# AnimatedRNG/alphazero-rs

Measured on AMD Instinct MI355X. Metric: selfplay_games_per_sec, higher is better.
Workload: dtype bf16

## Files before the change

alphazero-rs_amd/csrc/az_engine.hip:

```cpp
#include "../../include/az_engine.h"
#include "../../include/az_reanalyse.h"
#include "../../include/az_search_stop.h"

#include <dlfcn.h>
#include <unistd.h>
#include <rccl/rccl.h>

#include <algorithm>
#include <array>
#include <atomic>
#include <chrono>
#include <cstdio>
#include <cstring>
#include <map>
#include <memory>
#include <mutex>
#include <string>
#include <vector>

#include "az_combine.h"
#include "az_draw.h"
#include "az_local_comm.h"
#include "az_merge.h"
#include "az_net.h"
// ... 1120 lines not shown
    if (is("train_epochs") && value >= 1 && value <= 100000) { e->train_epochs = (int)value; return AZ_OK; }
    if (is("train_batch") && value >= 2 && value <= TRAIN_MAX_BATCH) { e->train_batch = (int)value; return AZ_OK; }
    if (is("train_seed")) { e->train_seed = (uint64_t)value; return AZ_OK; }
    if (is("train_graph") && (value == 0 || value == 1)) { e->train_graph = (int)value; if (e->trainer) trainer_set_graph(e->trainer, value != 0); return AZ_OK; }
    struct SwitchKey { const char* key; int TrainSwitches::* field; };
    static const SwitchKey switch_keys[] = {
        {"train_gemm", &TrainSwitches::gemm},
        {"train_fwd_dma", &TrainSwitches::fwd_dma},
        {"train_fwd_x3", &TrainSwitches::fwd_x3},
        {"train_wgrad_tr", &TrainSwitches::wgrad_tr},
        {"train_implicit", &TrainSwitches::implicit},
        {"train_gemm3_ring", &TrainSwitches::gemm3_ring},
        {"train_fork", &TrainSwitches::fork},
    };
    for (const SwitchKey& r : switch_keys) {
        if (!is(r.key) || (value != 0 && value != 1)) continue;
        e->train_sw.*r.field = (int)value;
        if (e->trainer) { (void)hipSetDevice(e->device); trainer_set_switches(e->trainer, e->train_sw); }
        return AZ_OK;
    }
    if (is("train_lr_e9") && value > 0) { e->hyper.lr = (float)((double)value * 1e-9); return AZ_OK; }
    if (is("train_dropout_e6") && value >= 0 && value < 1000000) { e->hyper.dropout = (float)((double)value * 1e-6); return AZ_OK; }
    if (is("train_keep_best") && (value == 0 || value == 1)) { e->train_keep_best = value; return AZ_OK; }
    if (is("train_patience")) {
        if (value < 0 || value > SCORE_MAX_PATIENCE) return fail(e, AZ_ERR_BAD_ARGUMENT, "train_patience must be in 0 .. 1000");
        e->train_patience = value;
        return AZ_OK;
    }
    struct OptimKey { const char* key; int64_t lo, hi; bool or_zero; int64_t az_engine::* field; const char* range; };
    static const OptimKey optim_keys[] = {
        {"train_weight_decay_e9", 0, OPTIM_WD_E9_MAX, false, &az_engine::train_weight_decay_e9, "train_weight_decay_e9 must be in 0 .. 1000000000"},
        {"train_clip_norm_e6", 1, OPTIM_CLIP_E6_MAX, true, &az_engine::train_clip_norm_e6, "train_clip_norm_e6 must be 0 or in 1 .. 1000000000000"},
        {"train_lr_warmup_steps", 0, OPTIM_STEPS_MAX, false, &az_engine::train_lr_warmup_steps, "train_lr_warmup_steps must be in 0 .. 2147483647"},
        {"train_lr_decay", 0, 2, false, &az_engine::train_lr_decay, "train_lr_decay must be 0, 1 or 2"},
        {"train_lr_floor_e6", 0, OPTIM_FLOOR_E6_MAX, false, &az_engine::train_lr_floor_e6, "train_lr_floor_e6 must be in 0 .. 1000000"},
        {"train_lr_total_steps", 0, OPTIM_STEPS_MAX, false, &az_engine::train_lr_total_steps, "train_lr_total_steps must be in 0 .. 2147483647"},
        {"train_ema_decay_e9", 1, OPTIM_EMA_E9_MAX, true, &az_engine::train_ema_decay_e9, "train_ema_decay_e9 must be 0 or in 1 .. 999999999"},
    };
    for (const OptimKey& r : optim_keys) {
        if (!is(r.key)) continue;
        if ((value < r.lo || value > r.hi) && !(r.or_zero && value == 0)) return fail(e, AZ_ERR_BAD_ARGUMENT, r.range);
        e->*r.field = value;
        return AZ_OK;
    }
#ifdef AZ_DIAG
    NetOptions& o = e->netopt;
    if (is("conv2_table") && value == 2) { o.conv2_table = 2; return AZ_OK; }
    if (is("gemm_variant") && (value == 0 || value == 1 || value == 2 || value == 3 || value == 5 || value == 13)) { o.gemm_variant = (int)value; return AZ_OK; }
    if (is("fc_ring") && value >= 0 && value <= 3) { o.fc_ring = (int)value; return AZ_OK; }
    if (is("ring_tile") && value >= 0 && value < 60000) { const int l = (int)(value / 10000); if (l >= 3 && l <= 5) o.ring_tile[l] = (int)(value % 10000); return AZ_OK; }
    if (is("conv3_ring") && value >= 0 && value <= 3) { o.conv3_ring = (int)value; return AZ_OK; }
    if (is("conv2_pipe") && (value == 0 || value == 1)) { o.conv2_pipe = (int)value; return AZ_OK; }
    if (is("conv3_pipe") && value >= 0 && value <= 3) { o.conv3_pipe = (int)value; return AZ_OK; }
    if (is("conv1_table") && (value == 0 || value == 1)) { o.conv1_table = (int)value; return AZ_OK; }
    if (is("conv4_big") && value >= 0 && value <= 2) { o.conv4_big = (int)value; return AZ_OK; }
    if (is("tree_stamps") && (value == 0 || value == 1)) { return tree_set_stamps((int)value) ? AZ_OK : fail(e, AZ_ERR_HIP, "tree_set_stamps"); }
    if (is("print_clock_stamps")) {
        auto it = e->nets.find((int)value);
        std::vector<unsigned long long> st(2048);
        if (it == e->nets.end() || !it->second.conv || !netws_read_clock_stamps(e->ws[0], st.data()))
            return fail(e, AZ_ERR_BAD_ARGUMENT, "no conv net under that model id");
        std::vector<double> mhz;
        for (int i = 0; i < 1024; ++i) if (st[2 * i + 1]) mhz.push_back(100.0 * (double)st[2 * i] / (double)st[2 * i + 1]);
        std::sort(mhz.begin(), mhz.end());
        if (mhz.empty()) return fail(e, AZ_ERR_BAD_ARGUMENT, "no stamps (run a forward with gemm_variant 13 first)");
        char buf[160];
        std::snprintf(buf, sizeof buf, "clock MHz min %.0f median %.0f max %.0f over %zu blocks", mhz.front(), mhz[mhz.size() / 2], mhz.back(), mhz.size());
        e->err = buf;
        return AZ_OK;
    }
    if (is("print_seg_stamps")) {
        std::vector<unsigned long long> st(2048);
        if (!e->ws[0] || !netws_read_clock_stamps(e->ws[0], st.data())) return fail(e, AZ_ERR_BAD_ARGUMENT, "no workspace");
        std::string out;
        for (int i = 0; i < 10; ++i) {
            std::vector<unsigned long long> v;
            for (int b = 0; b < 128; ++b) if (st[16 * b + 8]) v.push_back(st[16 * b + i]);
            if (v.empty()) return fail(e, AZ_ERR_BAD_ARGUMENT, "no stamps (run a forward with conv3_pipe 3 first)");
            std::sort(v.begin(), v.end());
            char buf[64];
            std::snprintf(buf, sizeof buf, "%s%llu", i ? " " : "", v[v.size() / 2]);
            out += buf;
        }
        e->err = out;
        return AZ_OK;
    }
    if (is("print_tree_stamps")) {
        std::vector<unsigned long long> st(4096 * 8);
        if (!tree_read_stamps(st.data())) return fail(e, AZ_ERR_BAD_ARGUMENT, "no stamps (set tree_stamps 1 and run a search first)");
        std::string out;
        for (int i = 0; i < 7; ++i) {
            std::vector<unsigned long long> v;
            for (int w = 0; w < 4096; ++w) if (st[(size_t)w * 8 + 6]) v.push_back(st[(size_t)w * 8 + i]);
            if (v.empty()) return fail(e, AZ_ERR_BAD_ARGUMENT, "no stamps yet");
            std::sort(v.begin(), v.end());
            char buf[96];
            std::snprintf(buf, sizeof buf, "%s%llu/%llu/%llu", i ? " " : "", v[v.size() / 10], v[v.size() / 2], v[v.size() * 9 / 10]);
            out += buf;
        }
        e->err = out;
        return AZ_OK;
    }
#else
    static const struct { const char* k; int64_t dflt; } diag_keys[] = {{"gemm_variant", 5}, {"fc_ring", 1}, {"conv3_ring", 0}, {"conv2_pipe", 1},
                                                                         {"conv3_pipe", 1}, {"conv1_table", 1}, {"conv4_big", 0}, {"tree_stamps", 0}};
    bool diag_key = is("print_clock_stamps") || is("print_seg_stamps") || is("print_tree_stamps") || (is("conv2_table") && value == 2);
// ... 2648 lines not shown
```

alphazero-rs_amd/csrc/az_net.h:

```cpp
#pragma once
#include "az_tree.h"

namespace az {

struct ConvNet;
struct NetWorkspace;

struct Layout {
    int C;
    int64_t conv_w[4], conv_b[4], conv_bn[4], fc_w[2], fc_b[2], fc_bn[2], pi_w, pi_b, v_w, v_b, total;
    explicit Layout(int c) : C(c) {
        int64_t o = 0;
        for (int l = 0; l < 4; ++l) {
            int cin = l == 0 ? 2 : C;
            conv_w[l] = o; o += 9ll * cin * C;
            conv_b[l] = o; o += C;
            conv_bn[l] = o; o += 4ll * C;
        }
        const int fin[2] = {6 * C, 1024}, fout[2] = {1024, 512};
        for (int l = 0; l < 2; ++l) {
            fc_w[l] = o; o += (int64_t)fin[l] * fout[l];
            fc_b[l] = o; o += fout[l];
            fc_bn[l] = o; o += 4ll * fout[l];
        }
        pi_w = o; o += 512 * 7; pi_b = o; o += 7;
        v_w = o; o += 512; v_b = o; o += 1;
        total = o;
    }
};


struct NetProfile {
    double conv2_ms = 0, conv2_flops = 0, total_ms = 0, total_flops = 0;
    double conv3_ms = 0, conv3_flops = 0;
    double conv4_ms = 0, conv4_flops = 0;
    double fc_ms = 0, fc_flops = 0;
    double rows = 0;
    double conv2_bytes = 0;
    uint64_t launches = 0;
};

void launch_net_fixture(const EvalBatch& eb, int kind, uint64_t salt, hipStream_t s);

ConvNet* convnet_create(int channels, const char** err);
void convnet_destroy(ConvNet* n);
NetWorkspace* netws_create(int channels, int max_batch, const char** err);
void netws_destroy(NetWorkspace* ws);
int64_t convnet_param_count(int channels);
bool convnet_set_params(ConvNet* n, const float* host_params, int64_t count);
bool convnet_get_params(const ConvNet* n, float* host_params, int64_t count);
void convnet_init_random(ConvNet* n, uint64_t seed);
void netws_resolve_profile(NetWorkspace* ws, NetProfile* prof);
bool netws_conv3_accounting(NetWorkspace* ws, unsigned long long out[2], bool reset);
struct NetOptions {
    int conv2_table = 1;
    int conv3_small = 1;
    int conv3_planes = 1;
    int ring_packed = 1;
    int conv3_tail = 1;
    int conv3_wreg = 1;
    int net_fp8 = 0;
    int narrow_rows = 32;
    int gemm_variant = 5;
    int conv1_table = 1;
    int conv2_pipe = 1;
    int conv3_pipe = 1;
    int conv3_ring = 0;
    int conv4_big = 0;
    int fc_ring = 1;
    int ring_tile[6] = {0, 0, 0, 0, 0, 0};
};
bool netws_read_clock_stamps(NetWorkspace* ws, unsigned long long* out2048);
long long netws_read_conv3_out(NetWorkspace* ws, int rows, void* out);
#ifdef AZ_DIAG
long long netws_read_act(NetWorkspace* ws, int layer, int rows, void* out);
long long convnet_read_conv_table(const ConvNet* n, int which, int first_row, int n_rows, void* out);
#endif
long long netws_read_conv3_out_fp8(NetWorkspace* ws, int rows, void* out);
long long netws_read_conv2_out_fp8(NetWorkspace* ws, int rows, void* out);
unsigned long long netws_fp8_skinny_launches(const NetWorkspace* ws);
bool convnet_build_fp8(ConvNet* n, NetWorkspace* ws, hipStream_t s);
bool convnet_fp8_scales(const ConvNet* n, float out[2]);
bool convnet_prepare(NetWorkspace* ws, const NetOptions& opt);
void convnet_forward(ConvNet* n, NetWorkspace* ws, const EvalBatch& eb, int n_rows_hint, int n_rows_typ, hipStream_t s, NetProfile* prof,
                     const NetOptions& opt);

}
```

alphazero-rs_amd/csrc/az_net.hip:

```cpp
#include "az_net.h"
#include "az_fp8.h"

#include <algorithm>
#include <cmath>
#include <cstring>
#include <vector>

namespace az {

constexpr int ACTIONS = ConnectFour::ACTIONS;

typedef __bf16 bf16x8 __attribute__((ext_vector_type(8)));
typedef float f32x4 __attribute__((ext_vector_type(4)));
typedef int i32x4 __attribute__((ext_vector_type(4)));
typedef int i32x8 __attribute__((ext_vector_type(8)));

__global__ void k_net_fixture(EvalBatch eb, int kind, uint64_t salt) {
    uint32_t i = blockIdx.x * blockDim.x + threadIdx.x;
    if (i >= *eb.n) return;
    float pi[ACTIONS], v;
    if (kind == 0) {
#pragma unroll
        for (int a = 0; a < ACTIONS; ++a) pi[a] = __fdiv_rn(1.0f, 7.0f);
        v = 1.0f;
// ... 715 lines not shown
                    const int rl = mt * 16 + frow;
                    float r0 = acc[mt][nt][0] + bv.x, r1 = acc[mt][nt][1] + bv.y, r2 = acc[mt][nt][2] + bv.z,
                          r3 = acc[mt][nt][3] + bv.w;
                    if (d.relu) { r0 = fmaxf(r0, 0.f); r1 = fmaxf(r1, 0.f); r2 = fmaxf(r2, 0.f); r3 = fmaxf(r3, 0.f); }
                    uint2 o;
                    o.x = pack_bf16x2(r0, r1);
                    o.y = pack_bf16x2(r2, r3);
                    *(uint2*)(smem + rl * EP_STRIDE + nl * 2) = o;
                }
            }
        }
        __syncthreads();
#pragma unroll
        for (int it = 0; it < 128 * 16 / 256; ++it) {
            const int idx = it * 256 + tid;
            const int rl = idx >> 4, c = idx & 15;
            const int ml = half * 128 + rl;
            const int m = b0 * 42 + ml;
            if (ml >= IMG_ROWS || m >= M) continue;
            *(uint4*)(d.out + (size_t)m * d.N + n0 + c * 8) = *(const uint4*)(smem + rl * EP_STRIDE + c * 16);
        }
        __syncthreads();
    }
}

constexpr int C3_PLANE_BYTES = 32768;
constexpr int C3_TAB_INV = 512;
constexpr int C3_TAB_RD = 9 * 2 * 16 * 8;
constexpr int WF3_STEP = 4096;
constexpr int WF3_PAD = 1;
constexpr int C3_NB = 12;

template <int NB, int IH, int IW, int MT, int NTW, bool PLANES = false, int WREG = 0>
struct ConvTile {
    static constexpr int OH = IH - 2, OW = IW - 2, OUT_PER = OH * OW, IN_PER = IH * IW;
    static constexpr int OUT_ROWS = NB * OUT_PER, IMG_R = NB * IN_PER;
    static constexpr int NCOL = 32 * NTW, WROWS = 16 * MT;
    static constexpr int IMG_BYTES = PLANES ? 2 * C3_PLANE_BYTES : (IMG_R * 128 + 1023) / 1024 * 1024;
    static constexpr int LDS_BYTES = IMG_BYTES + (WREG ? 0 : NCOL * 128);
    static constexpr int EP_STRIDE = NCOL * 2 + 16;
    static_assert(OUT_ROWS <= 2 * WROWS && IMG_R % 8 == 0 && MT % 2 == 0, "tile");
    static_assert(LDS_BYTES <= 81920, "two workgroups must fit a CU's 160 KiB");
    static_assert(OUT_ROWS * EP_STRIDE <= LDS_BYTES, "the output tile must fit the dead buffers");
};

template <int NB, int IH, int IW, int MT, int NTW, bool PLANES = false, int WREG = 0>
__device__ __forceinline__ void conv_valid_tile(const GemmDesc& d, unsigned char* smem, const int b0 , const int n0 ,
                                                const int n_boards) {
    using T = ConvTile<NB, IH, IW, MT, NTW, PLANES, WREG>;
    static_assert(!PLANES || (NB == C3_NB && IH == 6 && IW == 7 && MT == 8), "the cell maps are conv3's");
    constexpr int OUT_PER = T::OUT_PER, IN_PER = T::IN_PER, OUT_ROWS = T::OUT_ROWS, IMG_R = T::IMG_R, NCOL = T::NCOL, OW = T::OW;
    constexpr int IMG_BYTES = T::IMG_BYTES;
    constexpr int IPIECES = (IMG_R + 31) / 32, WPIECES = NCOL / 32;
    constexpr int MH = MT / 2;
    constexpr int NM = MH * NTW;
    const int M = n_boards * OUT_PER;
    const int C = d.cin;
    const int tid = threadIdx.x, lane = tid & 63;
    const int wave = __builtin_amdgcn_readfirstlane(tid >> 6);
    const int wr = wave >> 1, wc = wave & 1;
    const int lrow = lane >> 3;
    const int chunk = (lane & 7) ^ lrow;
    typedef __attribute__((address_space(3))) void* lds_ptr;
    const uint32_t i_ob = (uint32_t)((b0 * IN_PER + wave * 8 + lrow) * C + chunk * 8) * 2u;
    uint32_t i_obp[8];
    if constexpr (PLANES) {
#pragma unroll
        for (int j = 0; j < 8; ++j) {
            const uint32_t e = d.c3tab[j * 64 + wave * 16 + (lane >> 2)];
            i_obp[j] = (uint32_t)((b0 * IN_PER + (int)(e & 1023u)) * C + (int)((((uint32_t)lane & 3u) ^ ((e >> 10) & 3u)) << 4)) * 2u;
        }
    }
    const uint32_t w_ob = (uint32_t)((n0 + wave * 8 + lrow) * d.K + chunk * 8) * 2u;
    const uint32_t lds_img = (uint32_t)(uintptr_t)(lds_ptr)(smem + wave * 1024);
    const uint32_t lds_w = (uint32_t)(uintptr_t)(lds_ptr)(smem + IMG_BYTES + wave * 1024);
    const size_t i_stride = (size_t)64 * C, w_stride = (size_t)64 * d.K;
#define AZ_TDMA_W(kk_)                                                                                       \
    {                                                                                                        \
        const char* wbase = (const char*)(d.W + (kk_));                                                      \
        _Pragma("unroll") for (int q_ = 0; q_ < WPIECES; ++q_) lds_dma16(wbase + q_ * w_stride, w_ob, lds_w + q_ * 4096); \
    }
#define AZ_TDMA_IMG(cb_)                                                                                     \
    {                                                                                                        \
        const char* ibase = (const char*)(d.A + (cb_) * 64);                                                 \
        if constexpr (PLANES) {                                                                              \
            _Pragma("unroll") for (int q_ = 0; q_ < 16; ++q_) lds_dma16(ibase + (q_ >> 3) * 16, i_obp[q_ & 7], lds_img + q_ * 4096); \
        } else {                                                                                             \
            _Pragma("unroll") for (int q_ = 0; q_ < IPIECES; ++q_)                                           \
                if ((q_ * 4 + 3) * 8 + 7 < IMG_R || (q_ * 4 + wave) * 8 + 7 < IMG_R)                         \
                    lds_dma16(ibase + q_ * i_stride, i_ob, lds_img + q_ * 4096);                             \
        }                                                                                                    \
    }
    f32x4 acc[MT][NTW];
#pragma unroll
    for (int i = 0; i < MT; ++i)
#pragma unroll
        for (int jn = 0; jn < NTW; ++jn) acc[i][jn] = f32x4{0.f, 0.f, 0.f, 0.f};
    const int frow = lane & 15, fq = lane >> 4, fsw = lane & 7;
    int rbase[MT];
#pragma unroll
    for (int mt = 0; mt < MT; ++mt) {
        int ml = wr * T::WROWS + mt * 16 + frow;
        ml = ml < OUT_ROWS ? ml : 0;
        const int bl = ml / OUT_PER, p = ml - bl * OUT_PER, y = p / OW, x = p - y * OW;
        rbase[mt] = bl * IN_PER + y * IW + x;
    }
    const int b_row0 = IMG_BYTES + (wc * (16 * NTW) + frow) * 128;
    const int coffB0 = ((0 + fq) ^ fsw) << 4, coffB1 = ((4 + fq) ^ fsw) << 4;
    const uint4* rdtab = (const uint4*)(d.c3tab + C3_TAB_INV) + (wr * 16 + frow);
    const uint32_t lane_x = (((uint32_t)fq & 1u) << 15) | (((uint32_t)fq >> 1) << 4);
    uint32_t tq[4] = {0, 0, 0, 0}, ntq[4] = {0, 0, 0, 0};
    if constexpr (PLANES) { const uint4 v = rdtab[0]; tq[0] = v.x; tq[1] = v.y; tq[2] = v.z; tq[3] = v.w; }
#define AZ_TCELL(q_, mt_) ((((mt_) & 1) ? q_[(mt_) >> 1] >> 16 : q_[(mt_) >> 1] & 0xFFFFu) ^ lane_x)
#define AZ_TLDA(dst_, mt0_, ks_, dt_, q_)                                                                    \
    _Pragma("unroll") for (int i_ = 0; i_ < MH; ++i_) {                                                      \
        if constexpr (PLANES) {                                                                              \
            dst_[i_] = *(const bf16x8*)(smem + (AZ_TCELL(q_, (mt0_) + i_) ^ ((ks_) << 5)));                  \
        } else {                                                                                             \
            const int r_ = rbase[(mt0_) + i_] + (dt_);                                                       \
            dst_[i_] = *(const bf16x8*)(smem + r_ * 128 + ((((ks_) * 4 + fq) ^ (r_ & 7)) << 4));             \
        }                                                                                                    \
    }
#define AZ_TLDB(dst_, coff_)                                                                                 \
    _Pragma("unroll") for (int i_ = 0; i_ < NTW; ++i_)                                                       \
        dst_[i_] = *(const bf16x8*)(smem + b_row0 + i_ * 2048 + (coff_));
#define AZ_TMMA(mt0_, fb_, fa_)                                                                              \
    _Pragma("unroll") for (int i_ = 0; i_ < MH; ++i_)                                                        \
        _Pragma("unroll") for (int j_ = 0; j_ < NTW; ++j_)                                                   \
            acc[(mt0_) + i_][j_] = __builtin_amdgcn_mfma_f32_16x16x32_bf16(fb_[j_], fa_[i_], acc[(mt0_) + i_][j_], 0, 0, 0);
#define AZ_TSB __builtin_amdgcn_sched_barrier(0)
#define AZ_TMIX(nr_)                                                                                         \
    {                                                                                                        \
        constexpr int nmf_ = NM / (2 * (nr_)) > 1 ? NM / (2 * (nr_)) : 1;                                    \
        _Pragma("unroll") for (int g_ = 0; g_ < (nr_); ++g_) {                                               \
            __builtin_amdgcn_sched_group_barrier(0x008, nmf_, 0);                                            \
            __builtin_amdgcn_sched_group_barrier(0x100, 1, 0);                                               \
        }                                                                                                    \
        if (NM - nmf_ * (nr_) > 0) __builtin_amdgcn_sched_group_barrier(0x008, NM - nmf_ * (nr_), 0);        \
    }
    static_assert(NM >= NTW + MH, "a cluster must hold at least one MFMA per read of its region");
    bf16x8 faX[MH], faY[MH];
    const int ncb = C / 64;
    const int nk = ncb * 9;
    int cb = 0, tap = 0, dt = 0;
    if constexpr (WREG == 0) {
    AZ_TDMA_W(0);
    AZ_TDMA_IMG(0);
    asm volatile("s_waitcnt vmcnt(0)" ::: "memory");
    __syncthreads();
    bf16x8 fbX[NTW], fbY[NTW];
    AZ_TLDB(fbX, coffB0);
    AZ_TLDA(faX, 0, 0, 0, tq);
    for (int kt = 0; kt < nk; ++kt) {
        const bool sw = tap == 8;
        const int ntap = sw ? 0 : tap + 1, ncbi = sw ? cb + 1 : cb;
        const int nky = ntap / 3, ndt = nky * IW + (ntap - nky * 3);
        const int kk = kt + 1 < nk ? ntap * C + ncbi * 64 : 8 * C + cb * 64;
        if constexpr (PLANES) { const uint4 v = rdtab[ntap * 32]; ntq[0] = v.x; ntq[1] = v.y; ntq[2] = v.z; ntq[3] = v.w; }
        AZ_TLDB(fbY, coffB1);
        AZ_TLDA(faY, MH, 0, dt, tq);
        AZ_TMMA(0, fbX, faX);
        AZ_TMIX(NTW + MH);
        AZ_TSB;
        __builtin_amdgcn_s_waitcnt(0xC07F);
        __builtin_amdgcn_s_barrier();
        AZ_TSB;
        AZ_TDMA_W(kk);
        AZ_TLDA(faX, 0, 1, dt, tq);
        AZ_TMMA(MH, fbX, faY);
        AZ_TMIX(MH);
        AZ_TSB;
        AZ_TLDA(faY, MH, 1, dt, tq);
        AZ_TMMA(0, fbY, faX);
        AZ_TMIX(MH);
        AZ_TSB;
        __builtin_amdgcn_s_waitcnt(0xC07F);
        asm volatile("s_waitcnt vmcnt(0)" ::: "memory");
        __builtin_amdgcn_s_barrier();
        AZ_TSB;
        if (sw && ncbi < ncb) {
            AZ_TDMA_IMG(ncbi);
            asm volatile("s_waitcnt vmcnt(0)" ::: "memory");
            __builtin_amdgcn_s_barrier();
        }
        AZ_TSB;
        AZ_TLDB(fbX, coffB0);
        AZ_TLDA(faX, 0, 0, ndt, ntq);
        AZ_TMMA(MH, fbY, faY);
        AZ_TMIX(NTW + MH);
        AZ_TSB;
        tap = ntap; cb = ncbi; dt = ndt;
        if constexpr (PLANES) { tq[0] = ntq[0]; tq[1] = ntq[1]; tq[2] = ntq[2]; tq[3] = ntq[3]; }
    }
    } else {
        static_assert(PLANES && WREG == 1, "the ring needs the 64 KiB PLANES image (the epilogue's tile must fit it)");
        static_assert(NTW == 4 || NTW == 2, "a wave's columns are one 64-channel group of the packed copy, or half of one");
        const __amdgpu_buffer_rsrc_t wrs = __builtin_amdgcn_make_buffer_rsrc((void*)d.Wf, 0, (d.K * d.N + WF3_PAD * WF3_STEP) * 2, 0x00020000);
        uint32_t wfo = (uint32_t)(((n0 >> 6) + (NTW == 4 ? wc : 0)) * nk) * 8192u + (uint32_t)(NTW == 4 ? 0 : wc * 2) * 2048u;
        const uint32_t wlane = (uint32_t)lane * 16u;
        bf16x8 fwX[NTW], fwY[NTW];
#define AZ_TLDW(dst_, off_)                                                                                  \
    _Pragma("unroll") for (int j_ = 0; j_ < NTW; ++j_)                                                       \
        dst_[j_] = __builtin_bit_cast(bf16x8, __builtin_amdgcn_raw_buffer_load_b128(wrs, wlane, wfo + (uint32_t)((off_) + j_ * 2048), 0));
        AZ_TDMA_IMG(0);
        AZ_TLDW(fwX, 0);
        AZ_TLDW(fwY, 1024);
        asm volatile("s_waitcnt vmcnt(0)" ::: "memory");
        __syncthreads();
        AZ_TLDA(faX, 0, 0, 0, tq);
        for (int kt = 0; kt < nk; ++kt) {
            const bool sw = tap == 8;
            const int ntap = sw ? 0 : tap + 1, ncbi = sw ? cb + 1 : cb;
            const int nky = ntap / 3, ndt = nky * IW + (ntap - nky * 3);
            { const uint4 v = rdtab[ntap * 32]; ntq[0] = v.x; ntq[1] = v.y; ntq[2] = v.z; ntq[3] = v.w; }
            AZ_TLDA(faY, MH, 0, dt, tq);
            AZ_TMMA(0, fwX, faX);
            AZ_TMIX(MH);
            AZ_TSB;
            AZ_TLDA(faX, 0, 1, dt, tq);
            AZ_TMMA(MH, fwX, faY);
            AZ_TMIX(MH);
            AZ_TSB;
            AZ_TLDW(fwX, 8192);
            AZ_TLDA(faY, MH, 1, dt, tq);
            AZ_TMMA(0, fwY, faX);
            __builtin_amdgcn_sched_group_barrier(0x020, NTW, 0);
            AZ_TMIX(MH);
            AZ_TSB;
            if (sw && ncbi < ncb) {
                __builtin_amdgcn_s_waitcnt(0xC07F);
                __builtin_amdgcn_s_barrier();
                AZ_TDMA_IMG(ncbi);
                asm volatile("s_waitcnt vmcnt(0)" ::: "memory");
                __builtin_amdgcn_s_barrier();
            }
            AZ_TSB;
            AZ_TLDA(faX, 0, 0, ndt, ntq);
            AZ_TMMA(MH, fwY, faY);
            AZ_TMIX(MH);
            AZ_TSB;
            AZ_TLDW(fwY, 8192 + 1024);
            wfo += 8192u;
            AZ_TSB;
            tap = ntap; cb = ncbi; dt = ndt;
            tq[0] = ntq[0]; tq[1] = ntq[1]; tq[2] = ntq[2]; tq[3] = ntq[3];
        }
#undef AZ_TLDW
    }
#undef AZ_TDMA_W
#undef AZ_TDMA_IMG
#undef AZ_TLDA
#undef AZ_TCELL
#undef AZ_TLDB
#undef AZ_TMMA
#undef AZ_TSB
#undef AZ_TMIX
    constexpr int EP_STRIDE = T::EP_STRIDE;
    __builtin_amdgcn_s_waitcnt(0xC07F);
    __builtin_amdgcn_s_barrier();
#pragma unroll
    for (int nt = 0; nt < NTW; ++nt) {
        const int nl = wc * (16 * NTW) + nt * 16 + fq * 4;
        const float4 bv = *(const float4*)(d.bias + n0 + nl);
#pragma unroll
        for (int mt = 0; mt < MT; ++mt) {
            const int ml = wr * T::WROWS + mt * 16 + frow;
            if (ml >= OUT_ROWS) continue;
            float r0 = acc[mt][nt][0] + bv.x, r1 = acc[mt][nt][1] + bv.y, r2 = acc[mt][nt][2] + bv.z,
                  r3 = acc[mt][nt][3] + bv.w;
            if (d.relu) { r0 = fmaxf(r0, 0.f); r1 = fmaxf(r1, 0.f); r2 = fmaxf(r2, 0.f); r3 = fmaxf(r3, 0.f); }
            uint2 o;
            o.x = pack_bf16x2(r0, r1);
            o.y = pack_bf16x2(r2, r3);
            *(uint2*)(smem + ml * EP_STRIDE + nl * 2) = o;
        }
    }
    __syncthreads();
    constexpr int EP_CHUNKS = OUT_ROWS * (NCOL / 8);
#pragma unroll
    for (int it = 0; it < (EP_CHUNKS + 255) / 256; ++it) {
        const int idx = it * 256 + tid;
        const int ml = idx / (NCOL / 8), c = idx - ml * (NCOL / 8);
        const int m = b0 * OUT_PER + ml;
        if (idx >= EP_CHUNKS || m >= M) continue;
        *(uint4*)(d.out + (size_t)m * d.N + n0 + c * 8) = *(const uint4*)(smem + ml * EP_STRIDE + c * 16);
    }
}

constexpr int C3_TAIL = 128;
template <bool PLANES, int WREG>
__device__ __forceinline__ void conv3_auto_body(const GemmDesc& d, unsigned char* smem, const int full_grid, const int tail_wgs) {
    const int n_boards = (int)(*d.n_dev);
    if (n_boards * d.rows_per_sample <= d.m_min) return;
    if (blockIdx.x == 0 && threadIdx.x == 0 && d.acct && n_boards > 0) { atomicAdd(&d.acct[0], (unsigned long long)n_boards); atomicAdd(&d.acct[1], 1ull); }
    const int NT = d.N / 128;
    const int tiles8 = ((n_boards + C3_NB - 1) / C3_NB + 7) / 8 * 8;
    const int wid = tiles8 * NT;
    const int full_rounds = wid / 512 * 512, rem = wid - full_rounds;
    const bool cut = rem > 0 && rem <= tail_wgs;
    int id = blockIdx.x, half = -1;
    if (id >= full_grid) {
        if (!cut || id - full_grid >= rem) return;
        id = full_rounds + (id - full_grid);
        half = 1;
    } else if (cut && id >= full_rounds) {
        half = 0;
    }
    const int xcd = id & 7, j = id >> 3;
    const int ntile = j % NT, mtile = (j / NT) * 8 + xcd;
    const int b0 = mtile * C3_NB, n0 = ntile * 128;
    if (b0 >= n_boards) return;
    if (half < 0) conv_valid_tile<C3_NB, 6, 7, 8, 4, PLANES, WREG>(d, smem, b0, n0, n_boards);
    else conv_valid_tile<C3_NB, 6, 7, 8, 2, PLANES, WREG>(d, smem, b0, n0 + half * 64, n_boards);
}
template <int LAYER, bool PLANES>
__global__ __launch_bounds__(256, 2) void k_conv3_auto(const GemmDesc d, const int full_grid, const int tail_wgs ) {
    __shared__ __attribute__((aligned(16))) unsigned char smem[ConvTile<C3_NB, 6, 7, 8, 4, PLANES>::LDS_BYTES];
    conv3_auto_body<PLANES, 0>(d, smem, full_grid, tail_wgs);
}
template <int LAYER>
__global__ __launch_bounds__(256, 2) void k_conv3_auto_wreg(const GemmDesc d, const int full_grid, const int tail_wgs) {
    __shared__ __attribute__((aligned(16))) unsigned char smem[ConvTile<C3_NB, 6, 7, 8, 4, true, 1>::LDS_BYTES];
    conv3_auto_body<true, 1>(d, smem, full_grid, tail_wgs);
}

template <int MR, int NR, int D>
__device__ __forceinline__ void gemm_skinny_tile(const GemmDesc& d, const int M, const int mtile, const int ntile, const int lane) {
    const int m0 = mtile * (16 * MR), n0 = ntile * (16 * NR);
    const int frow = lane & 15, fq = lane >> 4;
    const uint16_t* a_ptr[MR];
    const uint16_t* w_ptr[NR];
#pragma unroll
    for (int i = 0; i < MR; ++i) {
        int m = m0 + i * 16 + frow;
        m = m < M ? m : M - 1;
        const int b = m / d.rows_per_sample, r = m - b * d.rows_per_sample;
        const int y = r / d.out_w, x = r - y * d.out_w;
        a_ptr[i] = d.A + (size_t)((b * d.in_h + y) * d.in_w + x) * d.in_c + fq * 8;
    }
#pragma unroll
    for (int j = 0; j < NR; ++j) w_ptr[j] = d.W + (size_t)(n0 + j * 16 + frow) * d.K + fq * 8;
    const int ntaps = d.K / d.cin;
    const int nk = d.K / GBK;
    int ks_tap = 0, ks_kx = 0;
    uint32_t ks_c0 = 0, ks_toff = 0, ks_kk = 0;
    bf16x8 fa0[D][MR], fa1[D][MR], fb0[D][NR], fb1[D][NR];
#define AZ_SLOAD(s_)                                                                                    \
    {                                                                                                   \
        _Pragma("unroll") for (int i_ = 0; i_ < MR; ++i_) {                                             \
            fa0[s_][i_] = *(const bf16x8*)(a_ptr[i_] + ks_toff); fa1[s_][i_] = *(const bf16x8*)(a_ptr[i_] + ks_toff + 32); }  \
        _Pragma("unroll") for (int j_ = 0; j_ < NR; ++j_) {                                             \
            fb0[s_][j_] = *(const bf16x8*)(w_ptr[j_] + ks_kk); fb1[s_][j_] = *(const bf16x8*)(w_ptr[j_] + ks_kk + 32); }      \
        ++ks_tap; ++ks_kx; ks_toff += (uint32_t)d.in_c; ks_kk += (uint32_t)d.cin;                       \
        if (ks_kx == d.tap_w) { ks_kx = 0; ks_toff += (uint32_t)((d.in_w - d.tap_w) * d.in_c); }        \
        if (ks_tap == ntaps) { ks_tap = 0; ks_kx = 0; ks_c0 += GBK; ks_toff = ks_c0; ks_kk = ks_c0; }   \
    }
#define AZ_SMMA(s_)                                                                                     \
    _Pragma("unroll") for (int i_ = 0; i_ < MR; ++i_)                                                   \
        _Pragma("unroll") for (int j_ = 0; j_ < NR; ++j_) {                                             \
            acc[i_][j_] = __builtin_amdgcn_mfma_f32_16x16x32_bf16(fb0[s_][j_], fa0[s_][i_], acc[i_][j_], 0, 0, 0); \
            acc[i_][j_] = __builtin_amdgcn_mfma_f32_16x16x32_bf16(fb1[s_][j_], fa1[s_][i_], acc[i_][j_], 0, 0, 0); \
        }
    f32x4 acc[MR][NR];
#pragma unroll
    for (int i = 0; i < MR; ++i)
#pragma unroll
        for (int j = 0; j < NR; ++j) acc[i][j] = f32x4{0.f, 0.f, 0.f, 0.f};
#pragma unroll
    for (int st = 0; st < D; ++st) AZ_SLOAD(st);
    for (int kt = D; kt < nk; kt += D) {
#pragma unroll
        for (int st = 0; st < D; ++st) { AZ_SMMA(st); AZ_SLOAD(st); }
    }
#pragma unroll
    for (int st = 0; st < D; ++st) AZ_SMMA(st);
#undef AZ_SLOAD
#undef AZ_SMMA
// ... 448 lines not shown
        }
        for (int a = 0; a < 7; ++a) b[a] = p[L.pi_b + a];
        b[7] = p[L.v_b];
        ok &= hipMemcpy(net->wh, w.data(), w.size() * 4, hipMemcpyHostToDevice) == hipSuccess;
        ok &= hipMemcpy(net->bh, b.data(), b.size() * 4, hipMemcpyHostToDevice) == hipSuccess;
    }
    return ok;
}

bool convnet_get_params(const ConvNet* n, float* host_params, int64_t count) {
    if (!n || (int64_t)n->params.size() != count) return false;
    std::memcpy(host_params, n->params.data(), (size_t)count * sizeof(float));
    return true;
}

void convnet_init_random(ConvNet* net, uint64_t seed) {
    const Layout L(net->C);
    const int C = net->C;
    std::vector<float> p((size_t)L.total, 0.0f);
    uint64_t ctr = 0;
    auto fill = [&](int64_t off, int64_t n, int fan_in, int fan_out) {
        const float lim = std::sqrt(6.0f / (float)(fan_in + fan_out));
        for (int64_t i = 0; i < n; ++i) {
            uint64_t r = rng_draw(seed, ctr++, 0, RNG_WEIGHTS);
            float u = (float)(uint32_t)(r >> 40) * (1.0f / 16777216.0f);
            p[(size_t)(off + i)] = (2.0f * u - 1.0f) * lim;
        }
    };
    auto bn_default = [&](int64_t off, int n) {
        for (int i = 0; i < n; ++i) { p[(size_t)(off + i)] = 1.0f; p[(size_t)(off + 3 * n + i)] = 1.0f; }
    };
    for (int l = 0; l < 4; ++l) {
        int cin = l == 0 ? 2 : C;
        fill(L.conv_w[l], 9ll * cin * C, 9 * cin, 9 * C);
        bn_default(L.conv_bn[l], C);
    }
    fill(L.fc_w[0], 6ll * C * 1024, 6 * C, 1024); bn_default(L.fc_bn[0], 1024);
    fill(L.fc_w[1], 1024ll * 512, 1024, 512); bn_default(L.fc_bn[1], 512);
    fill(L.pi_w, 512 * 7, 512, 7);
    fill(L.v_w, 512, 512, 1);
    convnet_set_params(net, p.data(), L.total);
}


static bool conv3_is_small(const GemmDesc& d, int rows_hint, int rows_typ) {
    return (rows_typ > 0 ? (long long)rows_typ * 115 / 100 : (long long)rows_hint) * d.rows_per_sample <= 8192;
}
template <bool TABLE>
static void launch_conv2_gemm(const GemmDesc& d, int rows_hint, hipStream_t s) {
    const int tiles = (rows_hint + IMG_NB - 1) / IMG_NB;
    const int t8 = (tiles + 7) / 8 * 8;
    hipLaunchKernelGGL((k_conv_same_pipe<1, TABLE>), dim3(t8 * (d.N / HBN2_)), dim3(256), 0, s, d);
}
static void launch_conv3_image(const GemmDesc& d, int rows_hint, hipStream_t s, bool tail, bool planes, bool wreg) {
    const int tiles = (rows_hint + C3_NB - 1) / C3_NB;
    const int t8 = (tiles + 7) / 8 * 8;
    const int full_grid = t8 * (d.N / 128), tail_wgs = tail ? C3_TAIL : 0;
    const dim3 grid(full_grid + tail_wgs), block(256);
    if (wreg && planes && d.Wf) hipLaunchKernelGGL((k_conv3_auto_wreg<2>), grid, block, 0, s, d, full_grid, tail_wgs);
    else if (planes) hipLaunchKernelGGL((k_conv3_auto<2, true>), grid, block, 0, s, d, full_grid, tail_wgs);
    else hipLaunchKernelGGL((k_conv3_auto<2, false>), grid, block, 0, s, d, full_grid, tail_wgs);
}

template <int LAYER, int F8 = 0>
static void launch_ring_auto(const GemmDesc& d, int rows_hint, int rows_typ, hipStream_t s, bool force_one_per_cu = false) {
    const int m_est = (int)((rows_typ > 0 ? (long long)rows_typ * 115 / 100 : (long long)rows_hint) * d.rows_per_sample), ncol = d.N / GBN;
    const bool conv = d.tap_w > 1;
    const int tile_max = conv ? 96 : 128;
    const int m_one = 256 / ncol * tile_max;
    const int m_bound = rows_hint * d.rows_per_sample;
    auto launch = [&](bool one_per_cu, const GemmDesc& dd, int m_cover) {
        const int bmin = one_per_cu ? 64 : 96;
        const int mtb = ((m_cover + bmin - 1) / bmin + 7) / 8 * 8;
        if constexpr (F8 != 0) {
            if (one_per_cu) hipLaunchKernelGGL((k_gemm_ring_f8<LAYER, 4, F8>), dim3(mtb * ncol), dim3(256), 0, s, dd);
            else hipLaunchKernelGGL((k_gemm_ring_f8<LAYER, 2, F8>), dim3(mtb * ncol), dim3(256), 0, s, dd);
        } else if (one_per_cu) hipLaunchKernelGGL((k_gemm_ring_auto<LAYER, 4>), dim3(mtb * ncol), dim3(256), 0, s, dd);
        else hipLaunchKernelGGL((k_gemm_ring_auto<LAYER, 2>), dim3(mtb * ncol), dim3(256), 0, s, dd);
    };
    if (!force_one_per_cu && !conv && m_bound > m_one && (long long)m_est * 100 >= (long long)m_one * 70 && (long long)m_est * 100 <= (long long)m_one * 140) {
        GemmDesc lo = d, hi = d;
        lo.m_hi = m_one;
        hi.m_min = std::max(d.m_min, m_one);
        launch(true, lo, std::min(m_bound, m_one));
        launch(false, hi, m_bound);
        return;
    }
    const bool one_per_cu = force_one_per_cu || m_bound <= m_one || (m_est + tile_max - 1) / tile_max * ncol <= 256;
    launch(one_per_cu, d, m_bound);
}

#ifdef AZ_DIAG
template <int LAYER>
static bool launch_gemm_diag(const GemmDesc& d, int rows_hint, int rows_typ, hipStream_t s, const NetOptions& o) {
    const int v = o.gemm_variant;
    if ((v == 3 || v == 5) && LAYER == 1 && d.N % HBN_ == 0 && d.cin % 64 == 0) {
        const int tiles = (rows_hint + IMG_NB - 1) / IMG_NB;
        const int t8 = (tiles + 7) / 8 * 8;
        if (v == 5 && o.conv2_pipe) return false;
        if (v == 5 && d.states) hipLaunchKernelGGL((k_conv_img2<LAYER, true>), dim3(t8 * (d.N / HBN2_)), dim3(256), 0, s, d);
        else if (v == 5) hipLaunchKernelGGL((k_conv_img2<LAYER>), dim3(t8 * (d.N / HBN2_)), dim3(256), 0, s, d);
        else hipLaunchKernelGGL((k_conv_img<LAYER>), dim3(t8 * (d.N / HBN_)), dim3(512), 0, s, d);
        return true;
    }
    const bool big = v >= 1 && (LAYER == 1 || LAYER == 2 || (LAYER == 3 && !o.ring_tile[3] && (o.conv4_big == 1 || (o.conv4_big == 2 && rows_typ >= 4096)))) &&
                     d.N % HBN_ == 0;
    if constexpr (LAYER == 2) if (v == 5 && o.conv3_ring) {
        const int mt = (rows_hint * d.rows_per_sample + GBM - 1) / GBM;
        const int mt8 = (mt + 7) / 8 * 8;
        if (o.conv3_ring == 3) launch_ring_auto<LAYER>(d, rows_hint, rows_typ, s, true);
        else if (o.conv3_ring == 2) hipLaunchKernelGGL((k_gemm_ring<LAYER, 4>), dim3(mt8 * (d.N / GBN)), dim3(256), 0, s, d);
// ... 48 lines not shown
        if (o.fc_ring == 2) {
            const int m_typ = (rows_typ > 0 ? rows_typ : rows_hint) * d.rows_per_sample, ncol = d.N / GBN;
            const bool conv = d.tap_w > 1;
            const int ns = (m_typ + (conv ? 95 : 127)) / (conv ? 96 : 128) * ncol <= 256 ? 4 : 2;
            switch (ring_pick_bm(m_typ, ncol, ns, conv) * 10 + ns) {
                case 644: ring(integral_constant<int, 64>{}, integral_constant<int, 4>{}); break;
                case 964: ring(integral_constant<int, 96>{}, integral_constant<int, 4>{}); break;
                case 1284: ring(integral_constant<int, 128>{}, integral_constant<int, 4>{}); break;
                case 962: ring(integral_constant<int, 96>{}, integral_constant<int, 2>{}); break;
                case 1602: ring(integral_constant<int, 160>{}, integral_constant<int, 2>{}); break;
                case 1922: ring(integral_constant<int, 192>{}, integral_constant<int, 2>{}); break;
                default: ring(integral_constant<int, 128>{}, integral_constant<int, 2>{}); break;
            }
            return true;
        }
        if (o.fc_ring == 1) return false;
        hipLaunchKernelGGL((k_gemm_ring<LAYER, 2>), dim3(grid), dim3(256), 0, s, d);
        return true;
    }
    hipLaunchKernelGGL(k_gemm_mfma<LAYER>, dim3(grid), dim3(256), 0, s, d);
    return true;
}
#endif

template <int LAYER>
static void launch_gemm(const GemmDesc& d, int rows_hint, int rows_typ, hipStream_t s, const NetOptions& o) {
#ifdef AZ_DIAG
    if (launch_gemm_diag<LAYER>(d, rows_hint, rows_typ, s, o)) return;
#endif
    GemmDesc dd = d;
    if constexpr (LAYER >= 2) if (o.narrow_rows > 0 && d.N % 32 == 0) {
        const int lim = o.narrow_rows * (LAYER == 2 ? 1 : LAYER == 3 ? 2 : 4);
        const int est = rows_typ > 0 ? rows_typ : rows_hint;
        if (est <= 16 * lim) {
            dd.m_max = lim * d.rows_per_sample;
            const int rows_cov = rows_hint < lim ? rows_hint : lim;
            const dim3 grid((unsigned)skinny_waves_max(rows_cov * d.rows_per_sample, d.N)), block(64);
            const int nk = d.K / GBK;
            if (nk % 8 == 0) hipLaunchKernelGGL((k_gemm_skinny<LAYER, 8>), grid, block, 0, s, dd);
            else if (nk % 6 == 0) hipLaunchKernelGGL((k_gemm_skinny<LAYER, 6>), grid, block, 0, s, dd);
            else hipLaunchKernelGGL((k_gemm_skinny<LAYER, 2>), grid, block, 0, s, dd);
            if (rows_hint <= lim) return;
            dd.m_min = dd.m_max;
        }
    }
    const GemmDesc& d2 = dd;
    if constexpr (LAYER == 1) if (d.N % HBN_ == 0 && d.cin % 64 == 0) {
        if (d.states) launch_conv2_gemm<true>(d2, rows_hint, s);
        else launch_conv2_gemm<false>(d2, rows_hint, s);
        return;
    }
    if constexpr (LAYER == 2) {
        if (o.conv3_small && conv3_is_small(d2, rows_hint, rows_typ)) launch_ring_auto<LAYER>(d2, rows_hint, rows_typ, s, true);
        else launch_conv3_image(d2, rows_hint, s, o.conv3_tail != 0, o.conv3_planes != 0, o.conv3_wreg != 0);
        return;
    }

    launch_ring_auto<LAYER>(d2, rows_hint, rows_typ, s);
}

template <int LAYER, int F8>
static void launch_gemm_f8(const GemmDesc& d, int rows_hint, int rows_typ, hipStream_t s, const NetOptions& o, NetWorkspace* ws) {
    GemmDesc dd = d;
    if (o.narrow_rows > 0 && d.N % 32 == 0 && d.cin % 128 == 0) {
        const int lim = o.narrow_rows * (LAYER == 2 ? 1 : 2);
        const int est = rows_typ > 0 ? rows_typ : rows_hint;
        if (est <= 16 * lim) {
            dd.m_max = lim * d.rows_per_sample;
            const int rows_cov = rows_hint < lim ? rows_hint : lim;
            const dim3 grid((unsigned)skinny_waves_max(rows_cov * d.rows_per_sample, d.N)), block(64);
            const int nk = d.K / 128;
            if (nk % 18 == 0) hipLaunchKernelGGL((k_gemm_skinny_f8<LAYER, F8, 9, 6>), grid, block, 0, s, dd);
            else hipLaunchKernelGGL((k_gemm_skinny_f8<LAYER, F8, 9, 3>), grid, block, 0, s, dd);
            ++ws->fp8_skinny_launches;
            if (rows_hint <= lim) return;
            dd.m_min = dd.m_max;
        }
    }
    launch_ring_auto<LAYER, F8>(dd, rows_hint, rows_typ, s);
}

unsigned long long netws_fp8_skinny_launches(const NetWorkspace* n) { return n ? n->fp8_skinny_launches : 0; }

static hipEvent_t net_event(NetWorkspace* n) {
    if (!n->ev_pool.empty()) { hipEvent_t e = n->ev_pool.back(); n->ev_pool.pop_back(); return e; }
    hipEvent_t e = nullptr;
    (void)hipEventCreate(&e);
    return e;
}

bool netws_conv3_accounting(NetWorkspace* n, unsigned long long out[2], bool reset) {
    if (!n || !n->acct) return true;
    unsigned long long h[2] = {0, 0};
    if (hipMemcpy(h, n->acct, sizeof h, hipMemcpyDeviceToHost) != hipSuccess) return false;
    out[0] += h[0]; out[1] += h[1];
    return !reset || hipMemset(n->acct, 0, sizeof h) == hipSuccess;
}

void netws_resolve_profile(NetWorkspace* n, NetProfile* prof) {
    if (!n) return;
    const int C = n->C;
    const double f_conv = 2.0 * 9.0 * C * C;
    const double per_sample = 2.0 * (42.0 * 18 * C) + f_conv * (42 + 20 + 6) + 2.0 * (6.0 * C * 1024 + 1024.0 * 512 + 512.0 * 8);
    if (!n->open.empty() && hipMemcpy(n->pinned_n, n->d_nlog, (size_t)n->pinned_next * sizeof(uint32_t), hipMemcpyDeviceToHost) != hipSuccess)
        prof = nullptr;
    for (auto& r : n->open) {
        float conv2 = 0, conv3 = 0, conv4 = 0, fcs = 0, total = 0;
// ... 287 lines not shown
```

Baseline: 10300.

## Give each conv3 wave a full-height column strip with register-held weights

Adds a WREG==2 path to the conv3 valid-conv tile. Each of the four waves now owns a 32-column strip across all rows (15x2 accumulators) instead of a 2x2 wave grid. Weights are streamed by buffer loads into double-buffered registers, and activation fragments are read from LDS with interleaved MFMA scheduling. The new path is the default for full tiles in the wreg kernel, while the old layout stays reachable through a diagnostic flag. The aim is to cut redundant weight traffic per wave and improve MFMA density, at the cost of more accumulator registers and more LDS activation reads per wave.

Result: no change. 10410, median of 6 (+1.0%).

```diff
diff --git a/alphazero-rs_amd/csrc/az_engine.hip b/alphazero-rs_amd/csrc/az_engine.hip
--- a/alphazero-rs_amd/csrc/az_engine.hip
+++ b/alphazero-rs_amd/csrc/az_engine.hip
@@ -1196,6 +1196,7 @@
     if (is("conv3_ring") && value >= 0 && value <= 3) { o.conv3_ring = (int)value; return AZ_OK; }
     if (is("conv2_pipe") && (value == 0 || value == 1)) { o.conv2_pipe = (int)value; return AZ_OK; }
     if (is("conv3_pipe") && value >= 0 && value <= 3) { o.conv3_pipe = (int)value; return AZ_OK; }
+    if (is("conv3_wcol") && (value == 0 || value == 1)) { o.conv3_wcol = (int)value; return AZ_OK; }
     if (is("conv1_table") && (value == 0 || value == 1)) { o.conv1_table = (int)value; return AZ_OK; }
     if (is("conv4_big") && value >= 0 && value <= 2) { o.conv4_big = (int)value; return AZ_OK; }
     if (is("tree_stamps") && (value == 0 || value == 1)) { return tree_set_stamps((int)value) ? AZ_OK : fail(e, AZ_ERR_HIP, "tree_set_stamps"); }
diff --git a/alphazero-rs_amd/csrc/az_net.h b/alphazero-rs_amd/csrc/az_net.h
--- a/alphazero-rs_amd/csrc/az_net.h
+++ b/alphazero-rs_amd/csrc/az_net.h
@@ -65,6 +65,7 @@
     int conv1_table = 1;
     int conv2_pipe = 1;
     int conv3_pipe = 1;
+    int conv3_wcol = 1;
     int conv3_ring = 0;
     int conv4_big = 0;
     int fc_ring = 1;
diff --git a/alphazero-rs_amd/csrc/az_net.hip b/alphazero-rs_amd/csrc/az_net.hip
--- a/alphazero-rs_amd/csrc/az_net.hip
+++ b/alphazero-rs_amd/csrc/az_net.hip
@@ -791,13 +791,14 @@
     constexpr int OUT_PER = T::OUT_PER, IN_PER = T::IN_PER, OUT_ROWS = T::OUT_ROWS, IMG_R = T::IMG_R, NCOL = T::NCOL, OW = T::OW;
     constexpr int IMG_BYTES = T::IMG_BYTES;
     constexpr int IPIECES = (IMG_R + 31) / 32, WPIECES = NCOL / 32;
-    constexpr int MH = MT / 2;
-    constexpr int NM = MH * NTW;
+    constexpr int AM = WREG == 2 ? 15 : MT, AN = WREG == 2 ? 2 : NTW;
+    constexpr int MH = WREG == 2 ? 5 : MT / 2;
+    constexpr int NM = MH * AN;
     const int M = n_boards * OUT_PER;
     const int C = d.cin;
     const int tid = threadIdx.x, lane = tid & 63;
     const int wave = __builtin_amdgcn_readfirstlane(tid >> 6);
-    const int wr = wave >> 1, wc = wave & 1;
+    const int wr = WREG == 2 ? 0 : wave >> 1, wc = WREG == 2 ? wave : wave & 1;
     const int lrow = lane >> 3;
     const int chunk = (lane & 7) ^ lrow;
     typedef __attribute__((address_space(3))) void* lds_ptr;
@@ -830,11 +831,11 @@
                     lds_dma16(ibase + q_ * i_stride, i_ob, lds_img + q_ * 4096);                             \
         }                                                                                                    \
     }
-    f32x4 acc[MT][NTW];
-#pragma unroll
-    for (int i = 0; i < MT; ++i)
-#pragma unroll
-        for (int jn = 0; jn < NTW; ++jn) acc[i][jn] = f32x4{0.f, 0.f, 0.f, 0.f};
+    f32x4 acc[AM][AN];
+#pragma unroll
+    for (int i = 0; i < AM; ++i)
+#pragma unroll
+        for (int jn = 0; jn < AN; ++jn) acc[i][jn] = f32x4{0.f, 0.f, 0.f, 0.f};
     const int frow = lane & 15, fq = lane >> 4, fsw = lane & 7;
     int rbase[MT];
 #pragma unroll
@@ -848,8 +849,9 @@
     const int coffB0 = ((0 + fq) ^ fsw) << 4, coffB1 = ((4 + fq) ^ fsw) << 4;
     const uint4* rdtab = (const uint4*)(d.c3tab + C3_TAB_INV) + (wr * 16 + frow);
     const uint32_t lane_x = (((uint32_t)fq & 1u) << 15) | (((uint32_t)fq >> 1) << 4);
-    uint32_t tq[4] = {0, 0, 0, 0}, ntq[4] = {0, 0, 0, 0};
+    uint32_t tq[WREG == 2 ? 8 : 4] = {}, ntq[WREG == 2 ? 8 : 4] = {};
     if constexpr (PLANES) { const uint4 v = rdtab[0]; tq[0] = v.x; tq[1] = v.y; tq[2] = v.z; tq[3] = v.w; }
+    if constexpr (WREG == 2) { const uint4 v = rdtab[16]; tq[4] = v.x; tq[5] = v.y; tq[6] = v.z; tq[7] = v.w; }
 #define AZ_TCELL(q_, mt_) ((((mt_) & 1) ? q_[(mt_) >> 1] >> 16 : q_[(mt_) >> 1] & 0xFFFFu) ^ lane_x)
 #define AZ_TLDA(dst_, mt0_, ks_, dt_, q_)                                                                    \
     _Pragma("unroll") for (int i_ = 0; i_ < MH; ++i_) {                                                      \
@@ -931,7 +933,7 @@
         tap = ntap; cb = ncbi; dt = ndt;
         if constexpr (PLANES) { tq[0] = ntq[0]; tq[1] = ntq[1]; tq[2] = ntq[2]; tq[3] = ntq[3]; }
     }
-    } else {
+    } else if constexpr (WREG == 1) {
         static_assert(PLANES && WREG == 1, "the ring needs the 64 KiB PLANES image (the epilogue's tile must fit it)");
         static_assert(NTW == 4 || NTW == 2, "a wave's columns are one 64-channel group of the packed copy, or half of one");
         const __amdgpu_buffer_rsrc_t wrs = __builtin_amdgcn_make_buffer_rsrc((void*)d.Wf, 0, (d.K * d.N + WF3_PAD * WF3_STEP) * 2, 0x00020000);
@@ -985,6 +987,76 @@
             tq[0] = ntq[0]; tq[1] = ntq[1]; tq[2] = ntq[2]; tq[3] = ntq[3];
         }
 #undef AZ_TLDW
+    } else {
+        static_assert(PLANES && NTW == 4 && MT == 8, "column strips are the full conv3 tile's");
+        const __amdgpu_buffer_rsrc_t wrs = __builtin_amdgcn_make_buffer_rsrc((void*)d.Wf, 0, (d.K * d.N + WF3_PAD * WF3_STEP) * 2, 0x00020000);
+        uint32_t wfo = (uint32_t)(((n0 >> 6) + (wc >> 1)) * nk) * 8192u + (uint32_t)((wc & 1) * 2) * 2048u;
+        const uint32_t wlane = (uint32_t)lane * 16u;
+        bf16x8 fwX[2], fwY[2];
+#define AZ_SLDW(dst_, off_)                                                                                  \
+    _Pragma("unroll") for (int j_ = 0; j_ < 2; ++j_)                                                         \
+        dst_[j_] = __builtin_bit_cast(bf16x8, __builtin_amdgcn_raw_buffer_load_b128(wrs, wlane, wfo + (uint32_t)((off_) + j_ * 2048), 0));
+#define AZ_SMMA(mt0_, fw_, fa_)                                                                              \
+    _Pragma("unroll") for (int i_ = 0; i_ < MH; ++i_)                                                        \
+        _Pragma("unroll") for (int j_ = 0; j_ < 2; ++j_)                                                     \
+            acc[(mt0_) + i_][j_] = __builtin_amdgcn_mfma_f32_16x16x32_bf16(fw_[j_], fa_[i_], acc[(mt0_) + i_][j_], 0, 0, 0);
+#define AZ_SSTEP()                                                                                           \
+    {                                                                                                        \
+        const bool sw = tap == 8;                                                                            \
+        const int ntap = sw ? 0 : tap + 1, ncbi = sw ? cb + 1 : cb;                                          \
+        const int nky = ntap / 3, ndt = nky * IW + (ntap - nky * 3);                                         \
+        { const uint4 v = rdtab[ntap * 32]; ntq[0] = v.x; ntq[1] = v.y; ntq[2] = v.z; ntq[3] = v.w; }        \
+        { const uint4 v = rdtab[ntap * 32 + 16]; ntq[4] = v.x; ntq[5] = v.y; ntq[6] = v.z; ntq[7] = v.w; }   \
+        AZ_TLDA(faY, MH, 0, dt, tq);                                                                         \
+        AZ_SMMA(0, fwX, faX);                                                                                \
+        AZ_TMIX(MH);                                                                                         \
+        AZ_TSB;                                                                                              \
+        AZ_TLDA(faX, 2 * MH, 0, dt, tq);                                                                     \
+        AZ_SMMA(MH, fwX, faY);                                                                               \
+        AZ_TMIX(MH);                                                                                         \
+        AZ_TSB;                                                                                              \
+        AZ_TLDA(faY, 0, 1, dt, tq);                                                                          \
+        AZ_SMMA(2 * MH, fwX, faX);                                                                           \
+        AZ_TMIX(MH);                                                                                         \
+        AZ_TSB;                                                                                              \
+        AZ_SLDW(fwX, 8192);                                   \
+        AZ_TLDA(faX, MH, 1, dt, tq);                                                                         \
+        AZ_SMMA(0, fwY, faY);                                                                                \
+        __builtin_amdgcn_sched_group_barrier(0x020, 2, 0);    \
+        AZ_TMIX(MH);                                                                                         \
+        AZ_TSB;                                                                                              \
+        AZ_TLDA(faY, 2 * MH, 1, dt, tq);                                                                     \
+        AZ_SMMA(MH, fwY, faX);                                                                               \
+        AZ_TMIX(MH);                                                                                         \
+        AZ_TSB;                                                                                              \
+        if (sw && ncbi < ncb) {                               \
+            __builtin_amdgcn_s_waitcnt(0xC07F);                                                              \
+            __builtin_amdgcn_s_barrier();                     \
+            AZ_TDMA_IMG(ncbi);                                                                               \
+            asm volatile("s_waitcnt vmcnt(0)" ::: "memory");  \
+            __builtin_amdgcn_s_barrier();                                                                    \
+        }                                                                                                    \
+        AZ_TSB;                                                                                              \
+        AZ_TLDA(faX, 0, 0, ndt, ntq);                         \
+        AZ_SMMA(2 * MH, fwY, faY);                                                                           \
+        AZ_TMIX(MH);                                                                                         \
+        AZ_TSB;                                                                                              \
+        AZ_SLDW(fwY, 8192 + 1024);                            \
+        wfo += 8192u;                                                                                        \
+        AZ_TSB;                                                                                              \
+        tap = ntap; cb = ncbi; dt = ndt;                                                                     \
+        _Pragma("unroll") for (int i_ = 0; i_ < 8; ++i_) tq[i_] = ntq[i_];                                   \
+    }
+        AZ_TDMA_IMG(0);
+        AZ_SLDW(fwX, 0);
+        AZ_SLDW(fwY, 1024);
+        asm volatile("s_waitcnt vmcnt(0)" ::: "memory");
+        __syncthreads();
+        AZ_TLDA(faX, 0, 0, 0, tq);
+        for (int kt = 0; kt < nk; ++kt) AZ_SSTEP();
+#undef AZ_SLDW
+#undef AZ_SMMA
+#undef AZ_SSTEP
     }
 #undef AZ_TDMA_W
 #undef AZ_TDMA_IMG
@@ -998,11 +1070,11 @@
     __builtin_amdgcn_s_waitcnt(0xC07F);
     __builtin_amdgcn_s_barrier();
 #pragma unroll
-    for (int nt = 0; nt < NTW; ++nt) {
-        const int nl = wc * (16 * NTW) + nt * 16 + fq * 4;
+    for (int nt = 0; nt < AN; ++nt) {
+        const int nl = wc * (16 * AN) + nt * 16 + fq * 4;
         const float4 bv = *(const float4*)(d.bias + n0 + nl);
 #pragma unroll
-        for (int mt = 0; mt < MT; ++mt) {
+        for (int mt = 0; mt < AM; ++mt) {
             const int ml = wr * T::WROWS + mt * 16 + frow;
             if (ml >= OUT_ROWS) continue;
             float r0 = acc[mt][nt][0] + bv.x, r1 = acc[mt][nt][1] + bv.y, r2 = acc[mt][nt][2] + bv.z,
@@ -1027,7 +1099,7 @@
 }
 
 constexpr int C3_TAIL = 128;
-template <bool PLANES, int WREG>
+template <bool PLANES, int WREG, int WFULL = WREG>
 __device__ __forceinline__ void conv3_auto_body(const GemmDesc& d, unsigned char* smem, const int full_grid, const int tail_wgs) {
     const int n_boards = (int)(*d.n_dev);
     if (n_boards * d.rows_per_sample <= d.m_min) return;
@@ -1049,7 +1121,7 @@
     const int ntile = j % NT, mtile = (j / NT) * 8 + xcd;
     const int b0 = mtile * C3_NB, n0 = ntile * 128;
     if (b0 >= n_boards) return;
-    if (half < 0) conv_valid_tile<C3_NB, 6, 7, 8, 4, PLANES, WREG>(d, smem, b0, n0, n_boards);
+    if (half < 0) conv_valid_tile<C3_NB, 6, 7, 8, 4, PLANES, WFULL>(d, smem, b0, n0, n_boards);
     else conv_valid_tile<C3_NB, 6, 7, 8, 2, PLANES, WREG>(d, smem, b0, n0 + half * 64, n_boards);
 }
 template <int LAYER, bool PLANES>
@@ -1060,8 +1132,15 @@
 template <int LAYER>
 __global__ __launch_bounds__(256, 2) void k_conv3_auto_wreg(const GemmDesc d, const int full_grid, const int tail_wgs) {
     __shared__ __attribute__((aligned(16))) unsigned char smem[ConvTile<C3_NB, 6, 7, 8, 4, true, 1>::LDS_BYTES];
-    conv3_auto_body<true, 1>(d, smem, full_grid, tail_wgs);
-}
+    conv3_auto_body<true, 1, 2>(d, smem, full_grid, tail_wgs);
+}
+#ifdef AZ_DIAG
+template <int LAYER>
+__global__ __launch_bounds__(256, 2) void k_conv3_auto_wreg22(const GemmDesc d, const int full_grid, const int tail_wgs) {
+    __shared__ __attribute__((aligned(16))) unsigned char smem[ConvTile<C3_NB, 6, 7, 8, 4, true, 1>::LDS_BYTES];
+    conv3_auto_body<true, 1, 1>(d, smem, full_grid, tail_wgs);
+}
+#endif
 
 template <int MR, int NR, int D>
 __device__ __forceinline__ void gemm_skinny_tile(const GemmDesc& d, const int M, const int mtile, const int ntile, const int lane) {
@@ -1616,11 +1695,15 @@
     const int t8 = (tiles + 7) / 8 * 8;
     hipLaunchKernelGGL((k_conv_same_pipe<1, TABLE>), dim3(t8 * (d.N / HBN2_)), dim3(256), 0, s, d);
 }
-static void launch_conv3_image(const GemmDesc& d, int rows_hint, hipStream_t s, bool tail, bool planes, bool wreg) {
+static void launch_conv3_image(const GemmDesc& d, int rows_hint, hipStream_t s, bool tail, bool planes, bool wreg, bool wcol) {
     const int tiles = (rows_hint + C3_NB - 1) / C3_NB;
     const int t8 = (tiles + 7) / 8 * 8;
     const int full_grid = t8 * (d.N / 128), tail_wgs = tail ? C3_TAIL : 0;
     const dim3 grid(full_grid + tail_wgs), block(256);
+#ifdef AZ_DIAG
+    if (wreg && planes && d.Wf && !wcol) hipLaunchKernelGGL((k_conv3_auto_wreg22<2>), grid, block, 0, s, d, full_grid, tail_wgs);
+    else
+#endif
     if (wreg && planes && d.Wf) hipLaunchKernelGGL((k_conv3_auto_wreg<2>), grid, block, 0, s, d, full_grid, tail_wgs);
     else if (planes) hipLaunchKernelGGL((k_conv3_auto<2, true>), grid, block, 0, s, d, full_grid, tail_wgs);
     else hipLaunchKernelGGL((k_conv3_auto<2, false>), grid, block, 0, s, d, full_grid, tail_wgs);
@@ -1775,7 +1858,7 @@
     }
     if constexpr (LAYER == 2) {
         if (o.conv3_small && conv3_is_small(d2, rows_hint, rows_typ)) launch_ring_auto<LAYER>(d2, rows_hint, rows_typ, s, true);
-        else launch_conv3_image(d2, rows_hint, s, o.conv3_tail != 0, o.conv3_planes != 0, o.conv3_wreg != 0);
+        else launch_conv3_image(d2, rows_hint, s, o.conv3_tail != 0, o.conv3_planes != 0, o.conv3_wreg != 0, o.conv3_wcol != 0);
         return;
     }
 
```
